# IIT-PAVIS/DiffAssemble

Measured on AMD Instinct MI355X. Metric: denoising steps/sec (900-piece dense graph, T=100), higher is better.
Workload: dtype bf16

## Files before the change

diffassemble_amd/_lib.py:

```python
import ctypes as C
import os

import torch

LIB_PATH = os.environ.get("DA_LIB_PATH") or os.path.join(os.path.dirname(os.path.abspath(__file__)), "lib", "libdiffassemble_hip.so")
DA_MAX_LAYERS = 8
ABI_VERSION = 19
PREC_F32, PREC_BF16 = 0, 1
VARIANT_2D, VARIANT_3D = 0, 1
ARCH_TRANSFORMER, ARCH_EXOPHORMER, ARCH_GCN = 0, 1, 2
MEAN_EPSILON, MEAN_START_X = 0, 1
ACT_NONE, ACT_GELU, ACT_LEAKY02 = 0, 1, 2
CONV_Q_PRESCALED, CONV_FOLDED_V32 = 1, 2
TRAIN_MMA_FP32, TRAIN_MMA_BF16 = 0, 1
TRAIN_BWD_ALL, TRAIN_BWD_EARLY, TRAIN_BWD_LATE = 0, 1, 2
DBG_COUNTERS = ("opt_gen_workgroups", "dense_fast_exits", "dual_gen_slabs", "opt_masked_gen_workgroups")
DBG_LAUNCH_COUNTERS = {"resident_launches": 4, "virtual_rows_in_launch": 5}
PROF_CLASSES = ("embed", "linear_mlp", "linear_qkvs", "attn_hidden", "attn_last", "head", "update", "conv_fused")

_fp = C.c_void_p
_FPL = _fp * DA_MAX_LAYERS


class DaWeights(C.Structure):
    _fields_ = [
        ("variant", C.c_int32), ("arch", C.c_int32), ("steps", C.c_int32), ("c_in", C.c_int32),
        ("c_out", C.c_int32), ("feat_dim", C.c_int32), ("hidden", C.c_int32), ("heads", C.c_int32),
        ("n_layers", C.c_int32), ("virt_nodes", C.c_int32),
        ("time_emb", _fp),
        ("pos_w0", _fp), ("pos_b0", _fp), ("pos_w1", _fp), ("pos_b1", _fp),
        ("mlp_w0", _fp), ("mlp_b0", _fp), ("mlp_w1", _fp), ("mlp_b1", _fp),
        ("conv_wq", _FPL), ("conv_bq", _FPL), ("conv_wk", _FPL), ("conv_bk", _FPL),
        ("conv_wv", _FPL), ("conv_bv", _FPL), ("conv_ws", _FPL), ("conv_bs", _FPL),
        ("virt_emb", _fp),
        ("head_w0", _fp), ("head_b0", _fp), ("head_w1", _fp), ("head_b1", _fp),
        ("head_r_w0", _fp), ("head_r_b0", _fp), ("head_r_w1", _fp), ("head_r_b1", _fp),
    ]


class DaGraph(C.Structure):
    _fields_ = [
        ("n_nodes", C.c_int32), ("n_real", C.c_int32), ("n_graphs", C.c_int32), ("dense", C.c_int32),
        ("n_edges", C.c_int64),
        ("row_ptr", _fp), ("col_src", _fp), ("edge_id", _fp), ("graph_ptr", _fp),
        ("max_graph_nodes", C.c_int32), ("n_pad", C.c_int32),
        ("pad_ptr", _fp), ("row_map", _fp),
        ("out_ptr", _fp), ("out_dst", _fp),
        ("hybrid", C.c_int32), ("band_degree", C.c_int32),
        ("mask", _fp), ("mask_ptr", _fp), ("irr_row_ptr", _fp), ("irr_col_src", _fp),
        ("slot_node", _fp), ("blk_class", _fp), ("blk_class_ptr", _fp), ("blk_class_stride", C.c_int32), ("reserved1", C.c_int32),
# ... 34 lines not shown
        ("feat_dim", C.c_int32), ("reserved0", C.c_int32),
        ("premap", _fp * PCD_STAGES), ("bn_a", _fp * PCD_STAGES), ("conv_b", _fp * PCD_STAGES),
        ("conv6", _fp), ("linear0", _fp),
    ]


PCD_TRAIN_LAYERS = 8


class DaPcdTrainWeights(C.Structure):
    _fields_ = [
        ("feat_dim", C.c_int32), ("reserved0", C.c_int32),
        ("premap", _fp * PCD_STAGES), ("bn_a", _fp * PCD_STAGES), ("conv_b", _fp * PCD_STAGES),
        ("conv6", _fp), ("linear0", _fp),
        ("gamma", _fp * PCD_TRAIN_LAYERS), ("beta", _fp * PCD_TRAIN_LAYERS),
        ("running_mean", _fp * PCD_TRAIN_LAYERS), ("running_var", _fp * PCD_TRAIN_LAYERS),
        ("momentum", C.c_float * PCD_TRAIN_LAYERS), ("eps", C.c_float * PCD_TRAIN_LAYERS),
        ("inv_wf", _fp * 2), ("inv_wd", _fp * 2),
    ]


class DaPcdTrainGrads(C.Structure):
    _fields_ = [
        ("wf", _fp * 6), ("wd", _fp * 6), ("gamma", _fp * 6), ("beta", _fp * 6),
        ("linear0_w", _fp), ("linear0_b", _fp), ("points", _fp),
    ]


class DaConfig(C.Structure):
    _fields_ = [(n, C.c_int32) for n in ("struct_bytes", "disable_mfma", "disable_dense", "disable_folds", "attn_level", "xpanel", "tail_next",
                                         "pair_split", "train_attn", "train_side_streams")]


PROTOTYPES = {
    "da_abi_version": (C.c_int, []),
    "da_last_error": (C.c_char_p, []),
    "da_config_get": (C.c_int, [C.POINTER(DaConfig)]),
    "da_config_set": (C.c_int, [C.POINTER(DaConfig)]),
    "da_build_flags": (C.c_int, []),
    "da_denoiser_create": (C.c_int, [C.POINTER(DaWeights), C.c_int, _fp, C.POINTER(_fp)]),
    "da_denoiser_destroy": (None, [_fp]),
    "da_denoiser_flags": (C.c_int, [_fp]),
    "da_gcn_dinv": (C.c_int, [C.POINTER(DaGraph), _fp, _fp]),
    "da_gcn_aggregate": (C.c_int, [C.c_int, C.POINTER(DaGraph), C.c_int, _fp, _fp, _fp, C.c_int, _fp, _fp]),
    "da_denoiser_workspace_bytes": (C.c_size_t, [_fp, C.POINTER(DaGraph)]),
    "da_denoiser_set_features": (C.c_int, [_fp, C.POINTER(DaGraph), _fp, _fp, C.c_size_t, _fp]),
    "da_denoiser_forward": (C.c_int, [_fp, C.POINTER(DaGraph), _fp, _fp, C.c_int64, _fp, _fp, C.c_int, _fp, _fp,
                                      C.c_size_t, _fp]),
    "da_ddim_step": (C.c_int, [C.POINTER(DaSchedule), C.c_int, C.c_int, C.c_int, C.c_int, _fp, _fp, _fp,
                               C.c_int64, C.c_int, C.c_int, C.c_float, _fp, _fp, _fp]),
    "da_ddpm_step": (C.c_int, [C.POINTER(DaSchedule), C.c_int, C.c_int, _fp, _fp, _fp, C.c_int64, _fp, _fp, _fp]),
    "da_sample_loop": (C.c_int, [_fp, C.POINTER(DaGraph), C.POINTER(DaSchedule), C.c_int, C.c_int, C.c_int,
                                 _fp, _fp, _fp, _fp, C.c_size_t, C.c_int, _fp]),
    "da_sample_loop_ex": (C.c_int, [_fp, C.POINTER(DaGraph), C.POINTER(DaSchedule), C.c_int, C.c_int, C.c_int,
                                    _fp, _fp, _fp, _fp, C.c_size_t, C.c_int, C.POINTER(DaLoopOpts), _fp]),
    "da_sample_loop_pair": (C.c_int, [_fp, C.POINTER(DaSchedule), C.c_int, C.c_int, C.c_int,
                                      C.POINTER(DaGraph), _fp, _fp, _fp, C.c_size_t,
                                      C.POINTER(DaGraph), _fp, _fp, _fp, C.c_size_t, _fp]),
    "da_sample_loop_pair_traj": (C.c_int, [_fp, C.POINTER(DaSchedule), C.c_int, C.c_int, C.c_int,
                                           C.POINTER(DaGraph), _fp, _fp, _fp, C.c_size_t,
                                           C.POINTER(DaGraph), _fp, _fp, _fp, C.c_size_t, _fp, _fp, C.c_size_t, _fp]),
    "da_sample_loop_pair_ex": (C.c_int, [_fp, C.POINTER(DaSchedule), C.c_int, C.c_int, C.c_int,
                                         C.POINTER(DaGraph), _fp, _fp, _fp, C.c_size_t,
                                         C.POINTER(DaGraph), _fp, _fp, _fp, C.c_size_t, _fp, _fp, C.c_size_t,
                                         C.POINTER(DaLoopOpts), _fp, C.c_size_t, _fp]),
    "da_profile_enable": (C.c_int, [_fp, C.c_int]),
    "da_profile_read": (C.c_int, [_fp, C.POINTER(C.c_float), C.POINTER(C.c_int32)]),
    "da_linear": (C.c_int, [C.c_int, C.c_int, C.c_int, C.c_int, _fp, C.c_int, _fp, _fp, C.c_int, _fp, _fp,
                            C.c_int, _fp]),
    "da_linear_packed_bytes": (C.c_size_t, [C.c_int, C.c_int, C.c_int]),
    "da_linear_pack": (C.c_int, [C.c_int, C.c_int, C.c_int, _fp, C.c_int, _fp, _fp]),
# ... 50 lines not shown
    "da_expander_mask": (C.c_int, [C.c_int, C.c_int, C.c_int, _fp, _fp, C.c_int, _fp, _fp]),
    "da_train_backward": (C.c_int, [C.POINTER(DaWeights), C.POINTER(DaWeights), C.POINTER(DaGraph), _fp, _fp, _fp, _fp,
                                    _fp, C.c_size_t, _fp]),
}

_lib = None


class DaError(RuntimeError):
    pass


def lib():
    global _lib
    if _lib is None:
        if not os.path.exists(LIB_PATH):
            raise DaError(
                f"{LIB_PATH} not found: build it with `python -c 'import __graft_entry__ as g; g.build()'` "
                "(hipcc --offload-arch=gfx950).  diffassemble_amd has no CPU / eager fallback.")
        h = C.CDLL(LIB_PATH)
        for name, (res, args) in PROTOTYPES.items():
            fn = getattr(h, name)
            fn.restype = res
            fn.argtypes = args
        if h.da_abi_version() != ABI_VERSION:
            raise DaError(f"ABI mismatch: library reports {h.da_abi_version()}")
        _lib = h
    return _lib


def config():
    c = DaConfig()
    check(lib().da_config_get(C.byref(c)))
    return c


def set_config(**fields):
    old = config()
    new = DaConfig.from_buffer_copy(old)
    for k, v in fields.items():
        if k == "struct_bytes" or k not in dict(DaConfig._fields_):
            raise DaError(f"da_config has no field {k!r}")
        setattr(new, k, int(v))
    check(lib().da_config_set(C.byref(new)))
    return old


def experiments_build():
    return bool(lib().da_build_flags() & 1)


def check(rc):
    if rc != 0:
        raise DaError(f"libdiffassemble_hip error {rc}: {lib().da_last_error().decode(errors='replace')}")


def ptr(t):
    return None if t is None else C.c_void_p(t.data_ptr())


def stream_ptr(device=None):
    return C.c_void_p(torch.cuda.current_stream(device).cuda_stream)
```

diffassemble_amd/csrc/da_api.hip:

```cpp
#include <stdarg.h>
#include <stdlib.h>
#include <string.h>

#include <utility>
#include <vector>

#include "da_common.h"
#include "da_internal.h"
#include "da_config.h"

namespace da {

static thread_local char g_err[1024] = "";

void set_error(const char *fmt, ...) {
    va_list ap;
    va_start(ap, fmt);
    vsnprintf(g_err, sizeof(g_err), fmt, ap);
    va_end(ap);
}

struct ConvW {
    void *w = nullptr;
    float *b = nullptr;
// ... 10 lines not shown
}
static int scale_block(float *p, int rows, int cols, int ld, float s, hipStream_t st) {
    const size_t n = (size_t)rows * cols;
    if (!n) return 0;
    k_scale_block<<<(unsigned)((n + 255) / 256), 256, 0, st>>>(p, rows, cols, ld, s);
    DA_LAUNCH_CHECK();
    return 0;
}
__global__ void k_fill_bias_rows(int prec, int rows, int cols, const float *bias, void *dst) {
    const size_t i = (size_t)blockIdx.x * blockDim.x + threadIdx.x;
    if (i >= (size_t)rows * cols) return;
    const float v = bias[i % cols];
    if (prec == DA_PREC_BF16) ((bf16_t *)dst)[i] = f2bf(v); else ((float *)dst)[i] = v;
}
__global__ void k_cfg_combine(size_t n, float wgt, float *cond, const float *unc) {
    const size_t i = (size_t)blockIdx.x * blockDim.x + threadIdx.x;
    if (i < n) cond[i] = (1.0f + wgt) * cond[i] - wgt * unc[i];
}
static bool q_prescale_on() { return !(cfg().disable_folds & DA_FOLD_QSCALE); }
static float q_scale_log2(int C) { return 1.4426950408889634f / sqrtf((float)C); }

struct LoopKey {
    da_graph g;
    da_schedule s;
    int mean_type, ratio, max_iters;
    const float *x_init;
    float *traj, *x_final;
    void *ws;
    size_t ws_bytes;
    da_loop_opts opts;
    size_t traj_stride;
    size_t noise_stride;
    da_config cfg;
};

}

using namespace da;

struct da_denoiser {
    int prec = 0, variant = 0, arch = 0, steps = 0, c_in = 0, c_out = 0, F = 0, D = 0, hidden = 0, heads = 0,
        n_layers = 0, V = 0, head_hidden = 0;
    float *time_emb = nullptr, *pos_w0 = nullptr, *pos_b0 = nullptr, *pos_w1 = nullptr, *pos_b1 = nullptr;
    void *mlp_w0 = nullptr, *mlp_w1 = nullptr;
    float *mlp_b0 = nullptr, *mlp_b1 = nullptr;
    ConvW conv[DA_MAX_LAYERS];
    void *virt_emb = nullptr;
    void *head_w0 = nullptr;
    float *head_b0 = nullptr;
    float *head_w1 = nullptr, *head_b1 = nullptr, *head_r_w1 = nullptr, *head_r_b1 = nullptr;
    bool fused_mlp2 = false;
    void *conv0c_w = nullptr;
    float *conv0c_b = nullptr;
    void *headc_w = nullptr;
    float *headc_b = nullptr;
    void *virt_qkvs = nullptr;
    void *conv0c_wd = nullptr, *virt_qkvs_d = nullptr;
    void *conv0c_wdp = nullptr, *convLf_wp = nullptr;
    void *conv0c_wqs = nullptr;
    float *conv0c_bd = nullptr;
    bool q_prescaled = false;
    bool lastfold = false;
    bool dense_only = false;
    void *convLf_w = nullptr;
    float *convLf_b = nullptr;
    void *skipc_w = nullptr;
// ... 748 lines not shown
        cur = nxt;
    }
    if (x_final && cur != x_final) DA_CHECK_HIP(hipMemcpyAsync(x_final, cur, bytes, hipMemcpyDeviceToDevice, st));
    return 0;
}

int da_sample_loop_ex(da_denoiser *d, const da_graph *g, const da_schedule *s, int mean_type, int inference_ratio,
                      int max_iters, const float *x_init, float *traj, float *x_final, void *workspace,
                      size_t workspace_bytes, int use_graph, const da_loop_opts *opts, void *stream) {
    DA_REQUIRE(d && g && s && x_init && workspace, "da_sample_loop: null argument");
    da_loop_opts o;
    memset(&o, 0, sizeof(o));
    if (opts) { o.sampler = opts->sampler; o.eta = opts->eta; o.cfg = opts->cfg; o.cfg_w = opts->cfg_w; o.noise = opts->noise; }
    DA_REQUIRE(o.sampler == 0 || o.sampler == 1, "da_sample_loop_ex: sampler must be 0 (DDIM) or 1 (DDPM)");
    DA_REQUIRE(!(o.sampler == 1 || o.eta > 0.f) || o.noise, "da_sample_loop_ex: eta > 0 / DDPM need the noise buffer");
    DA_REQUIRE(d->variant == DA_VARIANT_2D || (!o.cfg && o.sampler == 0 && o.eta == 0.f), "da_sample_loop_ex: the 3D loop has no guidance / stochastic variant");
    DA_REQUIRE(inference_ratio >= 1 && s->steps >= 1, "da_sample_loop: bad ratio/steps");
    DA_REQUIRE(d->variant == DA_VARIANT_3D || d->c_in == d->c_out, "da_sample_loop: c_in != c_out");
    int rc = check_graph(d, g);
    if (rc) return rc;
    Workspace w = carve(d, g, workspace);
    DA_REQUIRE(workspace_bytes >= w.total, "workspace too small: %zu < %zu", workspace_bytes, w.total);
    hipStream_t st = (hipStream_t)stream;
    int total = (s->steps + inference_ratio - 1) / inference_ratio;
    const int n_iters = (max_iters > 0 && max_iters < total) ? max_iters : total;
    if (d->prof_on) use_graph = 0;
    if (stream_is_capturing(st)) use_graph = 0;
    if (!use_graph) return enqueue_loop(d, g, s, mean_type, inference_ratio, n_iters, x_init, traj, x_final, w, st, &o);

    LoopKey key;
    memset(&key, 0, sizeof(key));
    key.g = *g; key.s = *s; key.mean_type = mean_type; key.ratio = inference_ratio; key.max_iters = n_iters;
    key.x_init = x_init; key.traj = traj; key.x_final = x_final; key.ws = workspace; key.ws_bytes = workspace_bytes;
    key.opts = o; key.cfg = cfg();
    hipGraphExec_t exec = nullptr;
    for (auto &e : d->loops)
        if (memcmp(&key, &e.key, sizeof(key)) == 0) exec = e.exec;
    if (!exec) {
        if (d->loops.size() >= 8) {
            (void)hipGraphExecDestroy(d->loops.front().exec);
            d->loops.erase(d->loops.begin());
        }
        hipGraph_t graph = nullptr;
        if (!d->cap_stream) DA_CHECK_HIP(hipStreamCreateWithFlags(&d->cap_stream, hipStreamNonBlocking));
        hipStream_t cs = d->cap_stream;
        DA_CHECK_HIP(hipStreamBeginCapture(cs, hipStreamCaptureModeRelaxed));
        rc = enqueue_loop(d, g, s, mean_type, inference_ratio, n_iters, x_init, traj, x_final, w, cs, &o);
        hipError_t e = hipStreamEndCapture(cs, &graph);
        if (rc) { if (graph) (void)hipGraphDestroy(graph); return rc; }
        if (e != hipSuccess || !graph) { set_error("hipStreamEndCapture failed: %s", hipGetErrorString(e)); return 2; }
        e = hipGraphInstantiate(&exec, graph, nullptr, nullptr, 0);
        (void)hipGraphDestroy(graph);
        if (e != hipSuccess) { set_error("hipGraphInstantiate failed: %s", hipGetErrorString(e)); return 2; }
        d->loops.push_back({key, exec});
    }
    DA_CHECK_HIP(hipGraphLaunch(exec, st));
    return 0;
}

int da_sample_loop(da_denoiser *d, const da_graph *g, const da_schedule *s, int mean_type, int inference_ratio,
                   int max_iters, const float *x_init, float *traj, float *x_final, void *workspace,
                   size_t workspace_bytes, int use_graph, void *stream) {
    return da_sample_loop_ex(d, g, s, mean_type, inference_ratio, max_iters, x_init, traj, x_final, workspace, workspace_bytes,
                             use_graph, nullptr, stream);
}

int da_sample_loop_pair_ex(da_denoiser *d, const da_schedule *s, int mean_type, int inference_ratio, int max_iters,
// ... 4 lines not shown
    DA_REQUIRE(d && s && g_a && g_b && x_init_a && x_init_b && x_final_a && x_final_b && workspace_a && workspace_b,
               "da_sample_loop_pair: null argument");
    da_loop_opts oa, ob;
    memset(&oa, 0, sizeof(oa));
    if (opts) { oa.sampler = opts->sampler; oa.eta = opts->eta; oa.cfg = opts->cfg; oa.cfg_w = opts->cfg_w; oa.noise = opts->noise; }
    ob = oa;
    ob.noise = noise_b;
    DA_REQUIRE(oa.sampler == 0 || oa.sampler == 1, "da_sample_loop_pair_ex: sampler must be 0 (DDIM) or 1 (DDPM)");
    DA_REQUIRE(!(oa.sampler == 1 || oa.eta > 0.f) || (oa.noise && ob.noise), "da_sample_loop_pair_ex: eta > 0 / DDPM need both noise pointers");
    DA_REQUIRE(d->variant == DA_VARIANT_2D || (!oa.cfg && oa.sampler == 0 && oa.eta == 0.f), "da_sample_loop_pair_ex: the 3D loop has no guidance / stochastic variant");
    DA_REQUIRE(inference_ratio >= 1 && s->steps >= 1, "da_sample_loop_pair: bad ratio/steps");
    DA_REQUIRE(d->variant == DA_VARIANT_3D || d->c_in == d->c_out, "da_sample_loop_pair: c_in != c_out");
    DA_REQUIRE((!g_a->hybrid && !g_b->hybrid) || da::cfg().pair_split, "da_sample_loop_pair: hybrid graphs need the two-graph form (da_config.pair_split = 1)");
    DA_REQUIRE(!d->prof_on, "da_sample_loop_pair: not available while profiling (event bracketing is not capturable)");
    DA_REQUIRE((traj_a == nullptr) == (traj_b == nullptr), "da_sample_loop_pair_traj: both trajectory pointers or none");
    DA_REQUIRE(!traj_a || traj_stride >= (size_t)(g_a->n_real + g_b->n_real) * (d->variant == DA_VARIANT_3D ? 7 : d->c_in),
               "da_sample_loop_pair_traj: traj_stride smaller than one iteration of both halves");
    int rc = check_graph(d, g_a);
    if (rc) return rc;
    if ((rc = check_graph(d, g_b))) return rc;
    const Workspace wa = carve(d, g_a, workspace_a), wb = carve(d, g_b, workspace_b);
    DA_REQUIRE(workspace_a_bytes >= wa.total && workspace_b_bytes >= wb.total, "da_sample_loop_pair: workspace too small");
    {
        const char *a0 = (const char *)workspace_a, *b0 = (const char *)workspace_b;
        DA_REQUIRE(a0 + wa.total <= b0 || b0 + wb.total <= a0, "da_sample_loop_pair: the two workspaces overlap");
    }
    const int total = (s->steps + inference_ratio - 1) / inference_ratio;
    const int n_iters = (max_iters > 0 && max_iters < total) ? max_iters : total;
    auto make_key = [&](const da_graph *g, const float *xi, float *xf, void *ws, size_t wsb, float *tr) {
        LoopKey k;
        memset(&k, 0, sizeof(k));
        k.g = *g; k.s = *s; k.mean_type = mean_type; k.ratio = inference_ratio; k.max_iters = n_iters;
        k.x_init = xi; k.traj = tr; k.x_final = xf; k.ws = ws; k.ws_bytes = wsb; k.traj_stride = tr ? traj_stride : 0;
        k.cfg = cfg();
        return k;
    };
    LoopKey ka = make_key(g_a, x_init_a, x_final_a, workspace_a, workspace_a_bytes, traj_a);
    LoopKey kb = make_key(g_b, x_init_b, x_final_b, workspace_b, workspace_b_bytes, traj_b);
    ka.opts = oa; kb.opts = ob;
    ka.noise_stride = oa.noise ? noise_stride : 0; kb.noise_stride = ob.noise ? noise_stride : 0;
    const int split_mode = cfg().pair_split;
    if (stream_is_capturing((hipStream_t)stream)) {
        hipStream_t us = (hipStream_t)stream;
        if (!d->pair_stream) {
            DA_CHECK_HIP(hipStreamCreateWithFlags(&d->pair_stream, hipStreamNonBlocking));
            DA_CHECK_HIP(hipEventCreateWithFlags(&d->ev_pair_fork, hipEventDisableTiming));
            DA_CHECK_HIP(hipEventCreateWithFlags(&d->ev_pair_join, hipEventDisableTiming));
        }
        hipStream_t ps = d->pair_stream;
        DA_CHECK_HIP(hipEventRecord(d->ev_pair_fork, us));
        DA_CHECK_HIP(hipStreamWaitEvent(ps, d->ev_pair_fork, 0));
        const int rca = enqueue_loop(d, g_a, s, mean_type, inference_ratio, n_iters, x_init_a, traj_a, x_final_a, wa, us, &oa, traj_stride, noise_stride);
        const int rcb = enqueue_loop(d, g_b, s, mean_type, inference_ratio, n_iters, x_init_b, traj_b, x_final_b, wb, ps, &ob, traj_stride, noise_stride);
        DA_CHECK_HIP(hipEventRecord(d->ev_pair_join, ps));
        DA_CHECK_HIP(hipStreamWaitEvent(us, d->ev_pair_join, 0));
        return rca ? rca : rcb;
    }
    hipGraphExec_t exec = nullptr, exec_b = nullptr;
    for (auto &e : d->pair_loops)
        if (memcmp(&ka, &e.a, sizeof(ka)) == 0 && memcmp(&kb, &e.b, sizeof(kb)) == 0 && (e.exec_b != nullptr) == (split_mode != 0)) { exec = e.exec; exec_b = e.exec_b; }
    if (!exec && split_mode) {
        if (d->pair_loops.size() >= 4) {
            (void)hipGraphExecDestroy(d->pair_loops.front().exec);
            if (d->pair_loops.front().exec_b) (void)hipGraphExecDestroy(d->pair_loops.front().exec_b);
            d->pair_loops.erase(d->pair_loops.begin());
        }
        if (!d->cap_stream) DA_CHECK_HIP(hipStreamCreateWithFlags(&d->cap_stream, hipStreamNonBlocking));
// ... 155 lines not shown
    int rc = 0;
    if (qsf) {
        if ((rc = pack_w_qs(heads, Din, (int)hc, w, wq_img, st))) return rc;
    } else
    rc = launch_gemm_mfma(prec, g->n_nodes, Din, nout, x, Din, w, b, DA_ACT_NONE, nullptr, nullptr, 0, &qs, st);
    DA_REQUIRE(rc == 0, "da_conv_dense_ex: projection shape (Din=%d, Nout=%d) not supported by the MFMA kernels", Din, nout);
    DenseLayout L;
    L.Q = qs.Q; L.K = qs.K; L.Vt = qs.Vt; L.S = qs.S; L.n_pad = g->n_pad; L.q_prescaled = (flags & DA_CONV_Q_PRESCALED) ? 1 : 0;
    if (qsf) { L.x = x; L.ldx = Din; L.kin = Din; L.wqs = wq_img; L.bias = b; }
    DenseFold fo;
    fo.cv = 32; fo.out = out; fo.n_rows = g->n_real;
    const DenseMask mk = dense_mask_of(g);
    rc = launch_attn_dense(prec, L, heads, C, g->n_graphs, g->max_graph_nodes, g->graph_ptr, g->pad_ptr, g->dense == 2, residual, act,
                           folded ? nullptr : out, st, g->hybrid ? &mk : nullptr, folded ? &fo : nullptr);
    DA_REQUIRE(rc == 0, "da_conv_dense_ex: attention launch failed (%d)", rc);
    return 0;
}

int da_debug_counters(int64_t *out, int n, int reset) {
    DA_REQUIRE(out && n >= DA_DBG_NCOUNTERS, "da_debug_counters: need room for %d counters", DA_DBG_NCOUNTERS);
    unsigned long long a[4] = {0, 0, 0, 0}, b2[2] = {0, 0};
    int rc;
    if ((rc = da::attn_dense_counters(a, reset))) return rc;
#ifdef DA_EXPERIMENTS
    if ((rc = da::attn_dual_counters(b2, reset))) return rc;
#endif
    for (int k = 0; k < n; ++k) out[k] = 0;
    out[DA_DBG_OPT_GEN_WORKGROUPS] = (int64_t)a[0];
    out[DA_DBG_DENSE_FAST_EXITS] = (int64_t)a[1];
    out[DA_DBG_DUAL_GEN_SLABS] = (int64_t)b2[0];
    out[DA_DBG_OPT_MASKED_GEN_WORKGROUPS] = (int64_t)a[2];
    out[DA_DBG_RES_LAUNCHES] = (int64_t)da::attn_res_launches(reset);
    out[DA_DBG_VIRT_IN_LAUNCH] = (int64_t)da::attn_virt_launches(reset);
    return 0;
}

int da_profile_enable(da_denoiser *d, int on) {
    DA_REQUIRE(d, "da_profile_enable: null denoiser");
    d->prof_on = on != 0;
    d->prof_used = 0;
    d->prof_cls.clear();
    return 0;
}

int da_profile_read(da_denoiser *d, float *ms, int32_t *counts) {
    DA_REQUIRE(d && ms && counts, "da_profile_read: null argument");
    for (int k = 0; k < DA_PROF_NCLASS; ++k) { ms[k] = 0.f; counts[k] = 0; }
    for (size_t k = 0; k < d->prof_cls.size(); ++k) {
        DA_CHECK_HIP(hipEventSynchronize(d->prof_ev[2 * k + 1]));
        float t = 0.f;
        DA_CHECK_HIP(hipEventElapsedTime(&t, d->prof_ev[2 * k], d->prof_ev[2 * k + 1]));
        ms[d->prof_cls[k]] += t;
        counts[d->prof_cls[k]] += 1;
    }
    d->prof_used = 0;
    d->prof_cls.clear();
    return 0;
}

int da_linear(int prec, int M, int K, int Nout, const void *A, int lda, const void *W, const float *bias, int act,
              const void *residual, void *out, int ldo, void *stream) {
    DA_REQUIRE(A && W && out, "da_linear: null argument");
    return da::linear(prec, M, K, Nout, A, lda, W, bias, act, residual, out, ldo, (hipStream_t)stream);
}

size_t da_linear_packed_bytes(int prec, int K, int Nout) {
// ... 35 lines not shown
```

diffassemble_amd/csrc/da_basic.hip:

```cpp
#include "da_common.h"
#include "da_internal.h"

namespace da {

template <typename T>
__global__ __launch_bounds__(256) void k_set_feats(int n, int F, int D, const float *__restrict__ feats,
                                                   T *__restrict__ comb_in) {
    size_t total = (size_t)n * F;
    for (size_t idx = (size_t)blockIdx.x * blockDim.x + threadIdx.x; idx < total;
         idx += (size_t)gridDim.x * blockDim.x) {
        size_t r = idx / F;
        int c = (int)(idx - r * F);
        stf(comb_in + r * D + c, feats[idx]);
    }
}

template <typename T>
__global__ __launch_bounds__(256) void k_set_virtual_rows(int rows, int V, int D, const T *__restrict__ emb,
                                                          T *__restrict__ dst) {
    size_t total = (size_t)rows * D;
    for (size_t idx = (size_t)blockIdx.x * blockDim.x + threadIdx.x; idx < total;
         idx += (size_t)gridDim.x * blockDim.x) {
        size_t r = idx / D;
        int c = (int)(idx - r * D);
// ... 443 lines not shown
            }
            const bf16_t *wp = (const bf16_t *)df.nx_wp;
            const bf16_t *fp = (const bf16_t *)df.nx_feat_proj + (size_t)row * 128;
            bf16_t *hn = (bf16_t *)df.nx_h + (size_t)row * 128;
#pragma unroll
            for (int mt = 0; mt < 4; ++mt) {
                tl_u32x4 wa[4];
#pragma unroll
                for (int c = 0; c < 4; ++c) wa[c] = *(const tl_u32x4 *)(wp + (size_t)(32 * mt + m) * df.nx_ldw + 16 * c + 8 * g);
                uint2 fpv[4];
#pragma unroll
                for (int q = 0; q < 4; ++q) fpv[q] = *(const uint2 *)(fp + 32 * mt + 8 * q + 4 * g);
                tl_f32x16 ac;
#pragma unroll
                for (int r = 0; r < 16; ++r) ac[r] = 0.f;
#pragma unroll
                for (int c = 0; c < 4; ++c)
                    ac = __builtin_amdgcn_mfma_f32_32x32x16_bf16(__builtin_bit_cast(tl_bf16x8, wa[c]), __builtin_bit_cast(tl_bf16x8, bx[c]), ac, 0, 0, 0);
#pragma unroll
                for (int q = 0; q < 4; ++q) {
                    float v[4] = {ac[4 * q] + bf2f((bf16_t)(fpv[q].x & 0xffff)), ac[4 * q + 1] + bf2f((bf16_t)(fpv[q].x >> 16)),
                                  ac[4 * q + 2] + bf2f((bf16_t)(fpv[q].y & 0xffff)), ac[4 * q + 3] + bf2f((bf16_t)(fpv[q].y >> 16))};
#pragma unroll
                    for (int e = 0; e < 4; ++e) v[e] = gelu_erf(v[e]);
                    if (row0 + m < n)
                        *(uint2 *)(hn + 32 * mt + 8 * q + 4 * g) = make_uint2((unsigned)f2bf(v[0]) | ((unsigned)f2bf(v[1]) << 16),
                                                                              (unsigned)f2bf(v[2]) | ((unsigned)f2bf(v[3]) << 16));
                }
            }
        }
    }
}

int launch_tail_fused(int prec, int n, int H, int c_out, int hidden, int din, const void *h, const void *xin, int ldx, const void *wh,
                      const float *bh, const void *wsk, const float *bsk, const void *pz, const float *w2, const float *b2, float *out,
                      hipStream_t st, DdimFuse *dfp) {
    const bool off = (cfg().disable_folds & DA_FOLD_TAIL) != 0;
    if (off || prec != DA_PREC_BF16 || hidden != 128 || din != 256 || H > 8 || c_out > 8 || (ldx & 7)) return -1;
    if (n <= 0) return 0;
    DdimFuse df;
    if (dfp) df = *dfp; else { df = DdimFuse(); df.x = nullptr; df.x_prev = nullptr; }
    const int slabs = (n + 31) / 32;
    int spw = (slabs + 1023) / 1024;
    spw = spw < 1 ? 1 : (spw > 4 ? 4 : spw);
    const bool nx_off = cfg().tail_next == 0;
    const bool next = dfp && df.x_prev && df.nx_on && !nx_off && df.nx_cin <= 8 && df.nx_cin == c_out && df.nx_h == h;
    if (next)
        k_tail_fused<true><<<(slabs + spw - 1) / spw, 64, 0, st>>>(n, H, c_out, (const bf16_t *)h, (const bf16_t *)xin, ldx, (const bf16_t *)wh, bh,
                                                                   (const bf16_t *)wsk, bsk, (const bf16_t *)pz, w2, b2, out, df, spw);
    else
        k_tail_fused<false><<<(slabs + spw - 1) / spw, 64, 0, st>>>(n, H, c_out, (const bf16_t *)h, (const bf16_t *)xin, ldx, (const bf16_t *)wh, bh,
                                                                    (const bf16_t *)wsk, bsk, (const bf16_t *)pz, w2, b2, out, df, spw);
    DA_LAUNCH_CHECK();
    if (next) dfp->nx_done = 1;
    return 0;
}

int launch_head_fold(int prec, int n, int H, int c_out, const void *pz, const void *pre, const float *w2, const float *b2,
                     float *out, hipStream_t st, const DdimFuse *dfp) {
    if (n <= 0) return 0;
    DdimFuse df;
    if (dfp) df = *dfp; else { df = DdimFuse(); df.x = nullptr; df.x_prev = nullptr; }
    if (c_out > 8) { set_error("launch_head_fold: c_out %d > 8", c_out); return 2; }
    if (prec == DA_PREC_BF16) k_head_fold<bf16_t><<<(n + 31) / 32, 256, 0, st>>>(n, H, c_out, (const bf16_t *)pz, (const bf16_t *)pre, w2, b2, out, df);
    else k_head_fold<float><<<(n + 31) / 32, 256, 0, st>>>(n, H, c_out, (const float *)pz, (const float *)pre, w2, b2, out, df);
    DA_LAUNCH_CHECK();
    return 0;
}


template <typename T>
__global__ __launch_bounds__(256) void k_scatter_virtual(int rows, int V, int H, int C, const T *__restrict__ src, int n_real,
                                                         const int32_t *__restrict__ row_map, size_t n_pad, T *Q, T *K, T *Vt,
                                                         T *S, T *qkvs) {
    const int HC = H * C;
    const size_t total = (size_t)rows * 4 * HC;
    for (size_t idx = (size_t)blockIdx.x * blockDim.x + threadIdx.x; idx < total; idx += (size_t)gridDim.x * blockDim.x) {
        const size_t r = idx / (4 * (size_t)HC);
        const int col = (int)(idx - r * 4 * HC), which = col / HC, f = col - which * HC;
        const T v = src[(size_t)(r % V) * 4 * HC + col];
// ... 26 lines not shown
```

diffassemble_amd/csrc/da_config.h:

```cpp
#pragma once
#include <stdlib.h>

#include "../../include/diffassemble_hip.h"

namespace da {

da_config &cfg();

enum { DA_FOLD_MLP2 = 1, DA_FOLD_LAST = 2, DA_FOLD_QSCALE = 4, DA_FOLD_DDIM = 8, DA_FOLD_TAIL = 16, DA_FOLD_HYBRID_OVERLAP = 32 };

#ifdef DA_EXPERIMENTS
inline int xenv_read(const char *name, int dflt) { const char *e = getenv(name); return e ? atoi(e) : dflt; }
#define DA_XENV(name, dflt) ([]() -> int { static const int v_ = da::xenv_read(name, dflt); return v_; }())
#define DA_XENV_LIVE(name) getenv(name)
#define DA_XENV_SET(name) (getenv(name) != nullptr)
#else
#define DA_XENV(name, dflt) (dflt)
#define DA_XENV_LIVE(name) ((const char *)nullptr)
#define DA_XENV_SET(name) (false)
#endif

}
```

diffassemble_amd/csrc/da_config.hip:

```cpp
#include <string.h>

#include <mutex>

#include "da_common.h"
#include "da_config.h"

namespace da {

static int env_or(const char *name, int dflt) { const char *e = getenv(name); return (e && e[0]) ? atoi(e) : dflt; }

static da_config load_env() {
    da_config c;
    memset(&c, 0, sizeof c);
    c.struct_bytes = (int)sizeof(da_config);
    c.disable_mfma = env_or("DA_DISABLE_MFMA", 0);
    c.disable_dense = env_or("DA_DISABLE_DENSE", 0);
    c.disable_folds = env_or("DA_DISABLE_FOLDS", 0);
    c.attn_level = env_or("DA_ATTN_LEVEL", 2);
    c.xpanel = env_or("DA_ENABLE_XPANEL", -1);
    c.tail_next = env_or("DA_TAIL_NEXT", -1);
    c.pair_split = env_or("DA_PAIR_SPLIT", 1);
    c.train_attn = env_or("DA_TRAIN_ATTN", 2);
    c.train_side_streams = env_or("DA_TRAIN_SIDE_STREAMS", 3);
    return c;
}

da_config &cfg() {
    static da_config c = load_env();
    return c;
}

}

extern "C" {

int da_config_get(da_config *out) {
    DA_REQUIRE(out, "da_config_get: null argument");
    *out = da::cfg();
    return 0;
}

int da_config_set(const da_config *in) {
    DA_REQUIRE(in && in->struct_bytes == (int)sizeof(da_config), "da_config_set: struct_bytes %d != %d (header / library mismatch)",
               in ? in->struct_bytes : -1, (int)sizeof(da_config));
    da::cfg() = *in;
    return 0;
}

int da_build_flags(void) {
#ifdef DA_EXPERIMENTS
    return 1;
#else
    return 0;
#endif
}

}
```

diffassemble_amd/csrc/da_internal.h:

```cpp
#pragma once
#include "da_common.h"
#include "da_config.h"

namespace da {

struct DeviceSchedule {
    int steps;
    const float *betas, *alphas_cumprod, *sqrt_recip_alphas, *sqrt_recip_alphas_cumprod,
        *sqrt_recipm1_alphas_cumprod, *sqrt_one_minus_alphas_cumprod, *posterior_variance;
};

__device__ __forceinline__ float ddim2d_value(const DeviceSchedule &s, int mean_type, long long ti, int ratio,
                                              int prev_all_nonneg, float eta, float xv, float m, float noise) {
    ti = ti < 0 ? 0 : (ti >= s.steps ? s.steps - 1 : ti);
    const long long tp = ti - ratio;
    const float ap = s.alphas_cumprod[ti];
    const float ap_prev = (prev_all_nonneg && tp >= 0) ? s.alphas_cumprod[tp] : 1.0f;
    const float beta = 1.0f - ap;
    const float x0 = mean_type == DA_MEAN_START_X ? m : (xv - sqrtf(beta) * m) / sqrtf(ap);
    const float eps = (s.sqrt_recip_alphas_cumprod[ti] * xv - x0) / s.sqrt_recipm1_alphas_cumprod[ti];
    const float var = ((1.0f - ap_prev) / (1.0f - ap)) * (1.0f - ap / ap_prev);
    const float std_eta = eta * sqrtf(var);
    float prev = sqrtf(ap_prev) * x0 + sqrtf(1.0f - ap_prev - std_eta * std_eta) * eps;
    if (eta > 0.f) prev += std_eta * noise;
// ... 120 lines not shown
    const uint8_t *blk_class = nullptr;
    const int64_t *blk_class_ptr = nullptr;
    int blk_class_stride = 0;
    const int32_t *rm_meta = nullptr;
    int v_rows = 0, v_n_real = 0;
    const int32_t *v_row_ptr = nullptr, *v_col_src = nullptr;
    const float *v_mult = nullptr;
    float *v_part = nullptr;
    unsigned *v_cnt = nullptr;
    int *v_taken = nullptr;
};
constexpr int DA_VIRT_SPLIT_MAX = 8;
inline DenseMask dense_mask_of(const da_graph *g) {
    DenseMask mk;
    mk.mask = g->mask; mk.mask_ptr = g->mask_ptr; mk.irr_row_ptr = g->irr_row_ptr; mk.irr_col_src = g->irr_col_src; mk.row_map = g->row_map;
    mk.slot_node = g->slot_node;
    mk.rm_meta = g->rm_meta;
    const bool cls = g->blk_class && g->blk_class_ptr && g->blk_class_stride > 0;
    mk.blk_class = cls ? g->blk_class : nullptr; mk.blk_class_ptr = cls ? g->blk_class_ptr : nullptr; mk.blk_class_stride = cls ? g->blk_class_stride : 0;
    return mk;
}
struct DenseFold {
    int cv;
    void *out;
    int n_rows;
};
int launch_attn_dense(int prec, const DenseLayout &L, int heads, int C, int n_graphs, int max_graph_nodes,
                      const int32_t *graph_ptr, const int32_t *pad_ptr, int nodiag, const void *res, int act,
                      void *out, hipStream_t st, const DenseMask *mk = nullptr, const DenseFold *fold = nullptr);
int launch_attn_dual(const DenseLayout &L, int heads, int C, int n_graphs, int max_graph_nodes, const int32_t *graph_ptr,
                     const int32_t *pad_ptr, int nodiag, int act, void *out, const DenseFold *fold, hipStream_t st);
int attn_dense_counters(unsigned long long *out4, int reset);
long long attn_virt_launches(int reset);
long long attn_res_launches(int reset);
int attn_dual_counters(unsigned long long *out2, int reset);
int launch_attn_csr_cont(int prec, int n_nodes, int n_real, const int32_t *irr_row_ptr, const int32_t *irr_col_src,
                         const int32_t *row_map, int heads, int C, int n_pad, const DenseLayout &L,
                         const void *residual, int act, void *out, hipStream_t st,
                         const float *mult = nullptr );

bool conv_fused_applicable(int prec, int heads, int C, int kin, int max_graph_nodes, int ldo);
int launch_conv_fused(int prec, int heads, int C, int kin, int n_graphs, int max_graph_nodes, const int32_t *graph_ptr,
                      int nodiag, const void *x, int ldx, const void *W, const float *bias, int act, void *out, int ldo,
                      hipStream_t st);

int pcd_knn_launch(int clouds, int N, int dim, const float *x, int ldx, int32_t *idx, const float *xn, hipStream_t st);
int pcd_premap_launch(int C, const float *X, int ldx, const float *Wm, long long total, float *T, hipStream_t st);
int pcd_edge_launch(const float *T, const int32_t *idx, const float *bn_a, const float *wb, int N, int clouds, float *Xout,
                    float *xn, hipStream_t st);
int pcd_conv6_final_launch(const float *X1, const float *X2, const float *X3, const float *w6, int feat, int N, int clouds,
                           float *partial, const float *lin0, int inv, float *out, int ldo, hipStream_t st);

int gcn_plan_kind(const da_graph *g);
int launch_gcn_dinv(const da_graph *g, float *dinv, hipStream_t st);
int launch_gcn_aggregate(int prec, const da_graph *g, int W, const float *dinv, const void *X, const float *bias, int act, void *out,
                         hipStream_t st);
int launch_gcn_aggregate_t(int prec, const da_graph *g, int W, const float *dinv, const void *X, void *out, hipStream_t st);
int launch_gcn_gelu_res(size_t n, const float *pre, const float *res, float *out, hipStream_t st);

int linear(int prec, int M, int K, int Nout, const void *A, int lda, const void *W, const float *bias, int act,
           const void *res, void *out, int ldo, hipStream_t st);

}
```

include/diffassemble_hip.h:

```cpp
#ifndef DIFFASSEMBLE_HIP_H
#define DIFFASSEMBLE_HIP_H

#include <stddef.h>
#include <stdint.h>

#ifdef __cplusplus
extern "C" {
#endif

#define DA_ABI_VERSION 19

enum { DA_PREC_F32 = 0, DA_PREC_BF16 = 1 };
enum { DA_VARIANT_2D = 0, DA_VARIANT_3D = 1 };
enum { DA_ARCH_TRANSFORMER = 0, DA_ARCH_EXOPHORMER = 1,
       DA_ARCH_GCN = 2 };
enum { DA_MEAN_EPSILON = 0, DA_MEAN_START_X = 1 };
enum { DA_ACT_NONE = 0, DA_ACT_GELU = 1, DA_ACT_LEAKY02 = 2 };
enum { DA_MAX_LAYERS = 8 };

int da_abi_version(void);
const char *da_last_error(void);

typedef struct da_config {
    int32_t struct_bytes;
    int32_t disable_mfma;
    int32_t disable_dense;
    int32_t disable_folds;
    int32_t attn_level;
    int32_t xpanel;
    int32_t tail_next;
    int32_t pair_split;
    int32_t train_attn;
    int32_t train_side_streams;
} da_config;
int da_config_get(da_config *out );
int da_config_set(const da_config *in );
int da_build_flags(void);

typedef struct da_weights {
    int32_t variant;
    int32_t arch;
    int32_t steps;
    int32_t c_in;
    int32_t c_out;
    int32_t feat_dim;
    int32_t hidden;
    int32_t heads;
    int32_t n_layers;
    int32_t virt_nodes;
    const float *time_emb;
    const float *pos_w0, *pos_b0;
    const float *pos_w1, *pos_b1;
    const float *mlp_w0, *mlp_b0;
    const float *mlp_w1, *mlp_b1;
    const float *conv_wq[DA_MAX_LAYERS], *conv_bq[DA_MAX_LAYERS];
    const float *conv_wk[DA_MAX_LAYERS], *conv_bk[DA_MAX_LAYERS];
    const float *conv_wv[DA_MAX_LAYERS], *conv_bv[DA_MAX_LAYERS];
    const float *conv_ws[DA_MAX_LAYERS], *conv_bs[DA_MAX_LAYERS];
    const float *virt_emb;
    const float *head_w0, *head_b0;
    const float *head_w1, *head_b1;
    const float *head_r_w0, *head_r_b0;
    const float *head_r_w1, *head_r_b1;
} da_weights;

typedef struct da_graph {
    int32_t n_nodes;
    int32_t n_real;
    int32_t n_graphs;
// ... 117 lines not shown
};
int da_profile_enable(da_denoiser *d, int on);
int da_profile_read(da_denoiser *d, float *ms ,
                    int32_t *counts );

int da_linear(int prec, int M, int K, int Nout, const void *A, int lda, const void *W,
              const float *bias, int act, const void *residual, void *out, int ldo, void *stream);

size_t da_linear_packed_bytes(int prec, int K, int Nout);
int da_linear_pack(int prec, int K, int Nout, const void *W, int ldw , void *packed, void *stream);
int da_linear_packed(int prec, int M, int K, int Nout, const void *A, int lda, const void *W, const void *packed,
                     const float *bias, int act, const void *residual, void *out, int ldo, void *stream);

int da_attn_csr(int prec, const da_graph *g, int heads, int C, const void *qkvs, const void *residual,
                int act, void *out, float *alpha, void *stream);

size_t da_attn_dense_scratch_bytes(int prec, const da_graph *g, int heads, int C);
int da_conv_dense(int prec, const da_graph *g, int heads, int C, int Din, const void *x, const void *w,
                  const float *b, const void *residual, int act, void *out, void *scratch, void *stream);

#define DA_CONV_Q_PRESCALED 1
#define DA_CONV_FOLDED_V32 2
int da_conv_dense_ex(int prec, const da_graph *g, int heads, int C, int Din, const void *x, const void *w,
                     const float *b, const void *residual, int act, void *out, void *scratch, int flags,
                     void *stream);

enum {
    DA_DBG_OPT_GEN_WORKGROUPS = 0,
    DA_DBG_DENSE_FAST_EXITS = 1,
    DA_DBG_DUAL_GEN_SLABS = 2,
    DA_DBG_OPT_MASKED_GEN_WORKGROUPS = 3,
    DA_DBG_RES_LAUNCHES = 4,
    DA_DBG_VIRT_IN_LAUNCH = 5,
    DA_DBG_NCOUNTERS = 8
};
int da_debug_counters(int64_t *out , int n, int reset);

size_t da_train_workspace_bytes(const da_weights *w, const da_graph *g);
size_t da_train_workspace_bytes_ex(const da_weights *w, const da_graph *g, int mma_precision);
#define DA_TRAIN_MMA_FP32 0
#define DA_TRAIN_MMA_BF16 1
int da_train_forward(const da_weights *w, const da_graph *g, const float *x, const int64_t *t,
                     const float *feats, float *out, void *workspace, size_t workspace_bytes,
                     void *stream);
int da_train_backward(const da_weights *w, const da_weights *grads, const da_graph *g, const float *x,
                      const int64_t *t, const float *d_out, float *d_feats, void *workspace,
                      size_t workspace_bytes, void *stream);
int da_train_forward_ex(const da_weights *w, const da_graph *g, const float *x, const int64_t *t,
                        const float *feats, float *out, void *workspace, size_t workspace_bytes,
                        int mma_precision, void *stream);
int da_train_backward_ex(const da_weights *w, const da_weights *grads, const da_graph *g, const float *x,
                         const int64_t *t, const float *d_out, float *d_feats, void *workspace,
                         size_t workspace_bytes, int mma_precision, void *stream);
#define DA_TRAIN_BWD_ALL 0
#define DA_TRAIN_BWD_EARLY 1
#define DA_TRAIN_BWD_LATE 2
int da_train_backward_stage(const da_weights *w, const da_weights *grads, const da_graph *g, const float *x,
                            const int64_t *t, const float *d_out, float *d_feats, void *workspace,
                            size_t workspace_bytes, int mma_precision, int stage, void *stream);

int da_q_sample(int steps, int n, int c, const float *sqrt_alphas_cumprod, const float *sqrt_one_minus_alphas_cumprod,
                const float *x_start, const float *noise, const int64_t *t, float *x_noisy, void *stream);
int da_loss_grad(int kind, size_t n, const float *target, const float *pred, float *loss, float *d_pred, void *stream);

int da_adafactor_step(int n_params, const void *param_table, int n_blocks, const void *block_table,
                      float *flat, const float *flat_grad, float *state, float *scratch,
// ... 110 lines not shown
```

Before: 94510.

## Add 4-wave workgroup tail kernel with warp-specialized weight staging and fused next-step MLP

Adds k_tail_wg, a 256-thread variant of the fused tail kernel. Three waves stage head and skip weights plus the next-step MLP weights into LDS while wave 0 prefetches row data and runs the MFMA chain, and then all four waves share the next-step embedding projection. It becomes the default when the next-step fusion applies (mode -1), replacing the single-wave k_tail_fused launch, with a runtime switch and a launch counter added. The intent is to spread per-slab weight loading and the next-step projection across waves instead of serializing them in one wave. The cost is more LDS and barriers per workgroup and possibly lower occupancy.

Result: no change. 95410 (median of 6 runs) (+1.0%).

```diff
diff --git a/diffassemble_amd/_lib.py b/diffassemble_amd/_lib.py
--- a/diffassemble_amd/_lib.py
+++ b/diffassemble_amd/_lib.py
@@ -15,7 +15,7 @@
 TRAIN_MMA_FP32, TRAIN_MMA_BF16 = 0, 1
 TRAIN_BWD_ALL, TRAIN_BWD_EARLY, TRAIN_BWD_LATE = 0, 1, 2
 DBG_COUNTERS = ("opt_gen_workgroups", "dense_fast_exits", "dual_gen_slabs", "opt_masked_gen_workgroups")
-DBG_LAUNCH_COUNTERS = {"resident_launches": 4, "virtual_rows_in_launch": 5}
+DBG_LAUNCH_COUNTERS = {"resident_launches": 4, "virtual_rows_in_launch": 5, "tail_wg_launches": 6}
 PROF_CLASSES = ("embed", "linear_mlp", "linear_qkvs", "attn_hidden", "attn_last", "head", "update", "conv_fused")
 
 _fp = C.c_void_p
@@ -116,11 +116,16 @@
                                          "pair_split", "train_attn", "train_side_streams")]
 
 
+EXTRA_SWITCHES = {"tail_wg": ("da_tail_wg_get", "da_tail_wg_set")}
+
+
 PROTOTYPES = {
     "da_abi_version": (C.c_int, []),
     "da_last_error": (C.c_char_p, []),
     "da_config_get": (C.c_int, [C.POINTER(DaConfig)]),
     "da_config_set": (C.c_int, [C.POINTER(DaConfig)]),
+    "da_tail_wg_get": (C.c_int, []),
+    "da_tail_wg_set": (C.c_int, [C.c_int]),
     "da_build_flags": (C.c_int, []),
     "da_denoiser_create": (C.c_int, [C.POINTER(DaWeights), C.c_int, _fp, C.POINTER(_fp)]),
     "da_denoiser_destroy": (None, [_fp]),
@@ -237,17 +242,28 @@
 def config():
     c = DaConfig()
     check(lib().da_config_get(C.byref(c)))
+    for k, (get, _) in EXTRA_SWITCHES.items():
+        setattr(c, k, int(getattr(lib(), get)()))
     return c
+
+
+def switch_names():
+    return [k for k, _ in DaConfig._fields_ if k != "struct_bytes"] + list(EXTRA_SWITCHES)
 
 
 def set_config(**fields):
     old = config()
     new = DaConfig.from_buffer_copy(old)
     for k, v in fields.items():
+        if k in EXTRA_SWITCHES:
+            continue
         if k == "struct_bytes" or k not in dict(DaConfig._fields_):
             raise DaError(f"da_config has no field {k!r}")
         setattr(new, k, int(v))
     check(lib().da_config_set(C.byref(new)))
+    for k, (_, put) in EXTRA_SWITCHES.items():
+        if k in fields:
+            getattr(lib(), put)(int(fields[k]))
     return old
 
 
diff --git a/diffassemble_amd/csrc/da_api.hip b/diffassemble_amd/csrc/da_api.hip
--- a/diffassemble_amd/csrc/da_api.hip
+++ b/diffassemble_amd/csrc/da_api.hip
@@ -66,6 +66,7 @@
     size_t traj_stride;
     size_t noise_stride;
     da_config cfg;
+    int tail_wg;
 };
 
 }
@@ -880,7 +881,7 @@
     memset(&key, 0, sizeof(key));
     key.g = *g; key.s = *s; key.mean_type = mean_type; key.ratio = inference_ratio; key.max_iters = n_iters;
     key.x_init = x_init; key.traj = traj; key.x_final = x_final; key.ws = workspace; key.ws_bytes = workspace_bytes;
-    key.opts = o; key.cfg = cfg();
+    key.opts = o; key.cfg = cfg(); key.tail_wg = tail_wg_mode();
     hipGraphExec_t exec = nullptr;
     for (auto &e : d->loops)
         if (memcmp(&key, &e.key, sizeof(key)) == 0) exec = e.exec;
@@ -951,7 +952,7 @@
         memset(&k, 0, sizeof(k));
         k.g = *g; k.s = *s; k.mean_type = mean_type; k.ratio = inference_ratio; k.max_iters = n_iters;
         k.x_init = xi; k.traj = tr; k.x_final = xf; k.ws = ws; k.ws_bytes = wsb; k.traj_stride = tr ? traj_stride : 0;
-        k.cfg = cfg();
+        k.cfg = cfg(); k.tail_wg = tail_wg_mode();
         return k;
     };
     LoopKey ka = make_key(g_a, x_init_a, x_final_a, workspace_a, workspace_a_bytes, traj_a);
@@ -1173,6 +1174,7 @@
     out[DA_DBG_OPT_MASKED_GEN_WORKGROUPS] = (int64_t)a[2];
     out[DA_DBG_RES_LAUNCHES] = (int64_t)da::attn_res_launches(reset);
     out[DA_DBG_VIRT_IN_LAUNCH] = (int64_t)da::attn_virt_launches(reset);
+    out[DA_DBG_TAIL_WG_LAUNCHES] = (int64_t)da::tail_wg_launches(reset);
     return 0;
 }
 
diff --git a/diffassemble_amd/csrc/da_basic.hip b/diffassemble_amd/csrc/da_basic.hip
--- a/diffassemble_amd/csrc/da_basic.hip
+++ b/diffassemble_amd/csrc/da_basic.hip
@@ -499,6 +499,233 @@
     }
 }
 
+template <bool NEXT>
+__global__ __launch_bounds__(256) __attribute__((amdgpu_waves_per_eu(4))) void k_tail_wg(
+    int n, int H, int c_out, const bf16_t *h, const bf16_t *__restrict__ xin, int ldx, const bf16_t *__restrict__ wh, const float *__restrict__ bh,
+    const bf16_t *__restrict__ wsk, const float *__restrict__ bsk, const bf16_t *__restrict__ pz, const float *__restrict__ w2,
+    const float *__restrict__ b2, float *__restrict__ out, DdimFuse df) {
+    constexpr int KH = 128, KX = 256, NCH = (KH + KX) / 16, NB = 4;
+    constexpr int NW_B0 = 128, NW_W1 = 144, NW_B1 = 656, NW_ALL = 688;
+    __shared__ tl_u32x4 s_w[NCH][64];
+    __shared__ tl_u32x4 s_bx[NEXT ? 4 : 1][64];
+    __shared__ float s_xn[32][9];
+    __shared__ float s_hid[NEXT ? 32 : 1][17];
+    __shared__ __attribute__((aligned(16))) float s_nw[NEXT ? NW_ALL : 4];
+    const int tid = threadIdx.x, w = __builtin_amdgcn_readfirstlane(tid >> 6), lane = tid & 63, m = lane & 31, g = lane >> 5;
+    const int row0 = blockIdx.x * 32;
+    const int row = min(row0 + m, n - 1);
+    const bool ddim = df.x_prev != nullptr;
+    const bf16_t *hrow = h + (size_t)row * KH + 8 * g, *xrow = xin + (size_t)row * ldx + 8 * g;
+#define TL_ROW_CHUNK(c) (*(const tl_u32x4 *)((c) < KH / 16 ? hrow + 16 * (c) : xrow + 16 * ((c) - KH / 16)))
+#define TL_MFMA_BATCH(b, xs)                                                                                                                        \
+    _Pragma("unroll") for (int c = 0; c < NB; ++c)                                                                                                \
+        acc = __builtin_amdgcn_mfma_f32_32x32x16_bf16(__builtin_bit_cast(tl_bf16x8, s_w[(b) * NB + c][lane]), __builtin_bit_cast(tl_bf16x8, xs[c]), acc, 0, 0, 0)
+#define TL_LOAD_BATCH(b, xs) _Pragma("unroll") for (int c = 0; c < NB; ++c) xs[c] = TL_ROW_CHUNK((b) * NB + c)
+#define TL_PZ_HEADS(pv, h0)                                                                                                                         \
+    _Pragma("unroll") for (int hh = 0; hh < 4; ++hh) _Pragma("unroll") for (int q = 0; q < 4; ++q) {                                              \
+        const uint2 u = *(const uint2 *)(pzrow + (size_t)max(min((h0) + hh, H - 1), 0) * n * 32 + 8 * q);                                           \
+        const unsigned keep = (unsigned)(((h0) + hh - H) >> 31);               \
+        pv[hh][q] = make_uint2(u.x & keep, u.y & keep);                                                                                             \
+    }
+    tl_u32x4 x0[NB], x1[NB], x2[NB];
+    tl_u32x4 wa[4];
+    uint2 fpv[4];
+    if (w == 0) {
+        TL_LOAD_BATCH(0, x0);
+        TL_LOAD_BATCH(1, x1);
+        TL_LOAD_BATCH(2, x2);
+    } else {
+        tl_u32x4 t[NCH / 3];
+#pragma unroll
+        for (int k = 0; k < NCH / 3; ++k) {
+            const int c = w - 1 + 3 * k;
+            t[k] = c < KH / 16 ? *(const tl_u32x4 *)(wh + (size_t)m * KH + 16 * c + 8 * g)
+                               : *(const tl_u32x4 *)(wsk + (size_t)m * KX + 16 * (c - KH / 16) + 8 * g);
+        }
+        if (ddim)
+            for (int i = tid - 64; i < 32 * c_out; i += 192) {
+                const int r = i / c_out, j = i - r * c_out;
+                s_xn[r][j] = df.x[(size_t)min(row0 + r, n - 1) * c_out + j];
+            }
+#pragma unroll
+        for (int k = 0; k < NCH / 3; ++k) s_w[w - 1 + 3 * k][lane] = t[k];
+    }
+    if (NEXT && w != 0) {
+        const int cin = df.nx_cin;
+        for (int i = tid - 64; i < NW_ALL; i += 192) {
+            float v;
+            if (i < NW_B0) v = i < 16 * cin ? df.nx_w0[i] : 0.f;
+            else if (i < NW_W1) v = df.nx_b0[i - NW_B0];
+            else if (i < NW_B1) v = df.nx_w1[i - NW_W1];
+            else v = df.nx_b1[i - NW_B1];
+            s_nw[i] = v;
+        }
+        if (w == 1) {
+            long long ti = df.nx_t;
+            ti = ti < 0 ? 0 : (ti >= df.nx_steps ? df.nx_steps - 1 : ti);
+#pragma unroll
+            for (int c = 0; c < 2; ++c) {
+                const f32x4_t *tr = (const f32x4_t *)(df.nx_time_emb + (size_t)ti * 32 + 16 * c + 8 * g);
+                const f32x4_t t0 = tr[0], t1 = tr[1];
+                s_bx[NEXT ? 2 + c : 0][lane] = (tl_u32x4){(unsigned)f2bf(t0[0]) | ((unsigned)f2bf(t0[1]) << 16), (unsigned)f2bf(t0[2]) | ((unsigned)f2bf(t0[3]) << 16),
+                                                           (unsigned)f2bf(t1[0]) | ((unsigned)f2bf(t1[1]) << 16), (unsigned)f2bf(t1[2]) | ((unsigned)f2bf(t1[3]) << 16)};
+            }
+        }
+    }
+    __syncthreads();
+    if (!NEXT && w != 0) return;
+    if (w == 0) {
+        tl_f32x16 acc;
+#pragma unroll
+        for (int r = 0; r < 16; ++r) { const int ch = (r & 3) + 8 * (r >> 2) + 4 * g; acc[r] = bh[ch] + bsk[ch]; }
+        const bf16_t *pzrow = pz + (size_t)row * 32 + 4 * g;
+        uint2 pza[4][4], pzb[4][4];
+        TL_MFMA_BATCH(0, x0); TL_LOAD_BATCH(3, x0);
+        __builtin_amdgcn_sched_barrier(0);
+        TL_MFMA_BATCH(1, x1); TL_LOAD_BATCH(4, x1);
+        __builtin_amdgcn_sched_barrier(0);
+        TL_MFMA_BATCH(2, x2); TL_LOAD_BATCH(5, x2);
+        __builtin_amdgcn_sched_barrier(0);
+        TL_PZ_HEADS(pza, 0);
+        TL_MFMA_BATCH(3, x0);
+        __builtin_amdgcn_sched_barrier(0);
+        TL_PZ_HEADS(pzb, 4);
+        TL_MFMA_BATCH(4, x1);
+        __builtin_amdgcn_sched_barrier(0);
+        TL_MFMA_BATCH(5, x2);
+        __builtin_amdgcn_sched_barrier(0);
+        float f[16];
+#pragma unroll
+        for (int r = 0; r < 16; ++r) f[r] = acc[r];
+#pragma unroll
+        for (int hb = 0; hb < 2; ++hb)
+#pragma unroll
+            for (int q = 0; q < 4; ++q)
+#pragma unroll
+                for (int hh = 0; hh < 4; ++hh) {
+                    const uint2 u = hb ? pzb[hh][q] : pza[hh][q];
+                    f[4 * q] += bf2f((bf16_t)(u.x & 0xffff)); f[4 * q + 1] += bf2f((bf16_t)(u.x >> 16));
+                    f[4 * q + 2] += bf2f((bf16_t)(u.y & 0xffff)); f[4 * q + 3] += bf2f((bf16_t)(u.y >> 16));
+                }
+        if (NEXT) {
+            const bf16_t *wp = (const bf16_t *)df.nx_wp;
+            const bf16_t *fp = (const bf16_t *)df.nx_feat_proj + (size_t)row * 128;
+#pragma unroll
+            for (int c = 0; c < 4; ++c) wa[c] = *(const tl_u32x4 *)(wp + (size_t)m * df.nx_ldw + 16 * c + 8 * g);
+#pragma unroll
+            for (int q = 0; q < 4; ++q) fpv[q] = *(const uint2 *)(fp + 8 * q + 4 * g);
+        }
+#pragma unroll
+        for (int r = 0; r < 16; ++r) f[r] = gelu_erf(f[r]);
+#pragma unroll
+        for (int j = 0; j < 8; ++j) {
+            if (j >= c_out) break;
+            float part = 0.f;
+#pragma unroll
+            for (int r = 0; r < 16; ++r) {
+                const int k0 = (r & 3) + 8 * (r >> 2);
+                const float wlo = w2[j * 32 + k0], whi = w2[j * 32 + k0 + 4];
+                part = fmaf(g ? whi : wlo, f[r], part);
+            }
+            const float a = b2[j] + part + __shfl_xor(part, 32);
+            const size_t o = (size_t)row * c_out + j;
+            float xn = 0.f;
+            if (ddim) xn = ddim2d_value(df.s, df.mean_type, df.t, df.ratio, df.prev_all_nonneg, 0.f, s_xn[m][j], a, 0.f);
+            if (g == 0) {
+                if (NEXT) s_xn[m][j] = xn;
+                if (row0 + m < n) {
+                    out[o] = a;
+                    if (ddim) df.x_prev[o] = xn;
+                }
+            }
+        }
+    }
+    else if (NEXT) {
+        const bf16_t *wp = (const bf16_t *)df.nx_wp;
+        const bf16_t *fp = (const bf16_t *)df.nx_feat_proj + (size_t)row * 128;
+#pragma unroll
+        for (int c = 0; c < 4; ++c) wa[c] = *(const tl_u32x4 *)(wp + (size_t)(32 * w + m) * df.nx_ldw + 16 * c + 8 * g);
+#pragma unroll
+        for (int q = 0; q < 4; ++q) fpv[q] = *(const uint2 *)(fp + 32 * w + 8 * q + 4 * g);
+    }
+    if (!NEXT) return;
+    __syncthreads();
+    const int pr = tid & 31, pp = tid >> 5;
+    {
+        const int cin = df.nx_cin;
+#pragma unroll
+        for (int z = 0; z < 2; ++z) {
+            const int u = 2 * pp + z;
+            float a = s_nw[NW_B0 + u];
+#pragma unroll
+            for (int j = 0; j < 8; ++j)
+                if (j < cin) a += s_nw[u * cin + j] * s_xn[pr][j];
+            s_hid[pr][u] = gelu_erf(a);
+        }
+    }
+    __syncthreads();
+    {
+        float hid[16];
+#pragma unroll
+        for (int k = 0; k < 16; ++k) hid[k] = s_hid[pr][k];
+        unsigned pk[2];
+#pragma unroll
+        for (int e2 = 0; e2 < 2; ++e2) {
+            unsigned short two[2];
+#pragma unroll
+            for (int z = 0; z < 2; ++z) {
+                const int o = 4 * pp + 2 * e2 + z;
+                const f32x4_t *wr = (const f32x4_t *)(s_nw + NW_W1 + o * 16);
+                float a = s_nw[NW_B1 + o];
+#pragma unroll
+                for (int q4 = 0; q4 < 4; ++q4) {
+                    const f32x4_t w4 = wr[q4];
+                    a += w4[0] * hid[4 * q4]; a += w4[1] * hid[4 * q4 + 1]; a += w4[2] * hid[4 * q4 + 2]; a += w4[3] * hid[4 * q4 + 3];
+                }
+                two[z] = f2bf(a);
+            }
+            pk[e2] = (unsigned)two[0] | ((unsigned)two[1] << 16);
+        }
+        ((uint2 *)&s_bx[NEXT ? pp >> 2 : 0][32 * ((pp >> 1) & 1) + pr])[pp & 1] = make_uint2(pk[0], pk[1]);
+    }
+    __syncthreads();
+    {
+        bf16_t *hn = (bf16_t *)df.nx_h + (size_t)row * 128;
+        tl_f32x16 ac;
+#pragma unroll
+        for (int r = 0; r < 16; ++r) ac[r] = 0.f;
+#pragma unroll
+        for (int c = 0; c < 4; ++c)
+            ac = __builtin_amdgcn_mfma_f32_32x32x16_bf16(__builtin_bit_cast(tl_bf16x8, wa[c]), __builtin_bit_cast(tl_bf16x8, s_bx[NEXT ? c : 0][lane]), ac, 0, 0, 0);
+#pragma unroll
+        for (int q = 0; q < 4; ++q) {
+            float v[4] = {ac[4 * q] + bf2f((bf16_t)(fpv[q].x & 0xffff)), ac[4 * q + 1] + bf2f((bf16_t)(fpv[q].x >> 16)),
+                          ac[4 * q + 2] + bf2f((bf16_t)(fpv[q].y & 0xffff)), ac[4 * q + 3] + bf2f((bf16_t)(fpv[q].y >> 16))};
+#pragma unroll
+            for (int e = 0; e < 4; ++e) v[e] = gelu_erf(v[e]);
+            if (row0 + m < n)
+                *(uint2 *)(hn + 32 * w + 8 * q + 4 * g) = make_uint2((unsigned)f2bf(v[0]) | ((unsigned)f2bf(v[1]) << 16),
+                                                                     (unsigned)f2bf(v[2]) | ((unsigned)f2bf(v[3]) << 16));
+        }
+    }
+}
+
+#undef TL_ROW_CHUNK
+#undef TL_MFMA_BATCH
+#undef TL_LOAD_BATCH
+#undef TL_PZ_HEADS
+
+static bool tail_wg_on(int mode, bool next, int n) {
+    (void)n;
+    return mode == 1 || (mode < 0 && next);
+}
+static long long g_tail_wg_launches = 0;
+long long tail_wg_launches(int reset) {
+    const long long v = g_tail_wg_launches;
+    if (reset) g_tail_wg_launches = 0;
+    return v;
+}
+
 int launch_tail_fused(int prec, int n, int H, int c_out, int hidden, int din, const void *h, const void *xin, int ldx, const void *wh,
                       const float *bh, const void *wsk, const float *bsk, const void *pz, const float *w2, const float *b2, float *out,
                       hipStream_t st, DdimFuse *dfp) {
@@ -512,7 +739,15 @@
     spw = spw < 1 ? 1 : (spw > 4 ? 4 : spw);
     const bool nx_off = cfg().tail_next == 0;
     const bool next = dfp && df.x_prev && df.nx_on && !nx_off && df.nx_cin <= 8 && df.nx_cin == c_out && df.nx_h == h;
-    if (next)
+    if (tail_wg_on(tail_wg_mode(), next, n)) {
+        if (next)
+            k_tail_wg<true><<<slabs, 256, 0, st>>>(n, H, c_out, (const bf16_t *)h, (const bf16_t *)xin, ldx, (const bf16_t *)wh, bh, (const bf16_t *)wsk, bsk,
+                                                   (const bf16_t *)pz, w2, b2, out, df);
+        else
+            k_tail_wg<false><<<slabs, 256, 0, st>>>(n, H, c_out, (const bf16_t *)h, (const bf16_t *)xin, ldx, (const bf16_t *)wh, bh, (const bf16_t *)wsk, bsk,
+                                                    (const bf16_t *)pz, w2, b2, out, df);
+        ++g_tail_wg_launches;
+    } else if (next)
         k_tail_fused<true><<<(slabs + spw - 1) / spw, 64, 0, st>>>(n, H, c_out, (const bf16_t *)h, (const bf16_t *)xin, ldx, (const bf16_t *)wh, bh,
                                                                    (const bf16_t *)wsk, bsk, (const bf16_t *)pz, w2, b2, out, df, spw);
     else
diff --git a/diffassemble_amd/csrc/da_config.h b/diffassemble_amd/csrc/da_config.h
--- a/diffassemble_amd/csrc/da_config.h
+++ b/diffassemble_amd/csrc/da_config.h
@@ -6,6 +6,7 @@
 namespace da {
 
 da_config &cfg();
+int &tail_wg_mode();
 
 enum { DA_FOLD_MLP2 = 1, DA_FOLD_LAST = 2, DA_FOLD_QSCALE = 4, DA_FOLD_DDIM = 8, DA_FOLD_TAIL = 16, DA_FOLD_HYBRID_OVERLAP = 32 };
 
diff --git a/diffassemble_amd/csrc/da_config.hip b/diffassemble_amd/csrc/da_config.hip
--- a/diffassemble_amd/csrc/da_config.hip
+++ b/diffassemble_amd/csrc/da_config.hip
@@ -30,6 +30,11 @@
     return c;
 }
 
+int &tail_wg_mode() {
+    static int m = -1;
+    return m;
+}
+
 }
 
 extern "C" {
@@ -47,6 +52,14 @@
     return 0;
 }
 
+int da_tail_wg_get(void) { return da::tail_wg_mode(); }
+
+int da_tail_wg_set(int mode) {
+    const int old = da::tail_wg_mode();
+    da::tail_wg_mode() = mode < 0 ? -1 : (mode ? 1 : 0);
+    return old;
+}
+
 int da_build_flags(void) {
 #ifdef DA_EXPERIMENTS
     return 1;
diff --git a/diffassemble_amd/csrc/da_internal.h b/diffassemble_amd/csrc/da_internal.h
--- a/diffassemble_amd/csrc/da_internal.h
+++ b/diffassemble_amd/csrc/da_internal.h
@@ -176,6 +176,7 @@
                      const int32_t *pad_ptr, int nodiag, int act, void *out, const DenseFold *fold, hipStream_t st);
 int attn_dense_counters(unsigned long long *out4, int reset);
 long long attn_virt_launches(int reset);
+long long tail_wg_launches(int reset);
 long long attn_res_launches(int reset);
 int attn_dual_counters(unsigned long long *out2, int reset);
 int launch_attn_csr_cont(int prec, int n_nodes, int n_real, const int32_t *irr_row_ptr, const int32_t *irr_col_src,
diff --git a/include/diffassemble_hip.h b/include/diffassemble_hip.h
--- a/include/diffassemble_hip.h
+++ b/include/diffassemble_hip.h
@@ -35,6 +35,8 @@
 } da_config;
 int da_config_get(da_config *out );
 int da_config_set(const da_config *in );
+int da_tail_wg_get(void);
+int da_tail_wg_set(int mode);
 int da_build_flags(void);
 
 typedef struct da_weights {
@@ -218,6 +220,7 @@
     DA_DBG_OPT_MASKED_GEN_WORKGROUPS = 3,
     DA_DBG_RES_LAUNCHES = 4,
     DA_DBG_VIRT_IN_LAUNCH = 5,
+    DA_DBG_TAIL_WG_LAUNCHES = 6,
     DA_DBG_NCOUNTERS = 8
 };
 int da_debug_counters(int64_t *out , int n, int reset);
```
